# CITlabRostock/citlab-article-separation-new

Hardware: AMD Instinct MI355X
Metric: newspaper pages/sec (ARU-Net seg + GNN relation) at 3000x4500 px (higher is better)
Workload: dtype f32s

## Files before the change

### citlab-article-separation-new_amd/_lib.py

```python
import ctypes as C
import os

_HERE = os.path.dirname(os.path.abspath(__file__))
LIB_PATH = os.path.join(_HERE, "csrc", "libasep_hip.so")


class AsepError(RuntimeError):
    pass


MLP_MAX_HIDDEN = 4
ABI_VERSION = 12


class _SizedCfg(C.Structure):

    def __init__(self, *args, **kw):
        super().__init__(C.sizeof(type(self)), *args, **kw)


class AruCfg(_SizedCfg):
    _fields_ = [(n, C.c_int32) for n in (
        "struct_size", "channels", "n_classes", "feat_root", "scale_space_num", "res_depth", "num_scales_att",
        "use_attention", "mvn", "apply_softmax", "compute_dtype", "activation", "plain_u", "input_pyramid", "inp4up")]
# ... 2 lines not shown
class GnnCfg(_SizedCfg):
    _fields_ = [(n, C.c_int32) for n in (
        "struct_size", "node_feature_dim", "edge_feature_dim", "num_transition_steps", "hidden_dim", "interaction_dim",
        "interaction_hidden", "cls_hidden1", "cls_hidden2", "num_classes", "undirected_graph", "compress_input_dim", "output_type", "attention_heads", "attention_merge", "attention_hidden",
        "aggregation_type", "interaction_hidden2", "interaction_hidden3", "interaction_hidden4", "attention_hidden2", "attention_hidden3",
        "attention_hidden4", "cls_hidden3", "cls_hidden4", "lstm_use_hidden", "lstm_use_input", "visual_edge_dims")]


class ClusterSetting(C.Structure):
    _fields_ = [("min_neighbors", C.c_int32), ("assign_noise", C.c_int32), ("conf_thr", C.c_double), ("agree_thr", C.c_double)]


RESIZE_MODES = {"keep": 0, "luma": 1}
EDGE_RULES = {"bb": 0, "line": 1}
SEP_ORIENTATIONS = {None: 0, "horizontal": 1, "vertical": 2}
JPEG_ORDERS = {"gray": 0, "bgr": 1, "rgb": 2}
CLUSTER_METHODS = {"dbscan": 0, "dbscan_std": 1, "greedy": 2}


class ClusterMethodSetting(C.Structure):
    _fields_ = [("method", C.c_int32), ("count", C.c_int32), ("assign_noise", C.c_int32), ("reserved", C.c_int32),
                ("conf_thr", C.c_double), ("param", C.c_double)]


class GnnPage(C.Structure):
    _fields_ = [("N", C.c_int32), ("E", C.c_int32), ("R", C.c_int32), ("d_edges", C.c_void_p), ("d_node_feat", C.c_void_p),
                ("d_edge_feat", C.c_void_p), ("d_image", C.c_void_p), ("d_regions", C.c_void_p), ("d_num_points", C.c_void_p),
                ("d_edge_regions", C.c_void_p), ("d_edge_num_points", C.c_void_p), ("d_relations", C.c_void_p), ("d_probs_out", C.c_void_p)]


class GnnPageU8(C.Structure):
    _fields_ = [("page", GnnPage), ("d_scan", C.c_void_p), ("src_h", C.c_int32), ("src_w", C.c_int32), ("src_c", C.c_int32)]


_P = C.c_void_p
SIGNATURES = {
    "asep_device_count": (C.c_int, []),
    "asep_init": (C.c_int, [C.c_int]),
    "asep_last_error": (C.c_char_p, []),
    "asep_version": (C.c_char_p, []),
    "asep_abi_version": (C.c_int, []),
    "asep_engine_switches": (C.c_char_p, []),
    "asep_aru_load": (_P, [_P, C.c_size_t, C.POINTER(AruCfg)]),
    "asep_aru_free": (None, [_P]),
    "asep_aru_forward": (C.c_int, [_P, _P, C.c_int, C.c_int, _P, _P, _P, C.c_float]),
    "asep_aru_forward_dev": (C.c_int, [_P, _P, C.c_int, C.c_int, _P, _P, _P, C.c_float, _P]),
    "asep_aru_forward_batch_dev": (C.c_int, [_P, C.c_int, _P, C.c_int, C.c_int, _P, _P, _P, C.c_float, _P]),
    "asep_aru_trim": (C.c_int, [_P]),
    "asep_aru_forward_batch_dev2": (C.c_int, [_P, C.c_int, _P, _P, _P, _P, _P, _P, C.c_float, _P]),
    "asep_aru_get_endpoint": (C.c_long, [_P, C.c_char_p, _P, C.c_size_t, C.POINTER(C.c_int32)]),
    "asep_aru_profile": (C.c_int, [_P, C.c_int]),
    "asep_aru_profile_report": (C.c_long, [_P, C.c_char_p, C.c_size_t]),
    "asep_aru_flops": (C.c_double, [_P, C.c_int, C.c_int]),
    "asep_host_alloc": (_P, [C.c_size_t]),
    "asep_host_free": (None, [_P]),
    "asep_host_register": (C.c_int, [_P, C.c_size_t]),
    "asep_host_unregister": (C.c_int, [_P]),
    "asep_gnn_load": (_P, [_P, C.c_size_t, C.POINTER(GnnCfg)]),
    "asep_gnn_free": (None, [_P]),
    "asep_gnn_correct_edges": (C.c_int, [_P, C.c_int, C.c_int, _P, _P, _P, _P]),
    "asep_gnn_forward": (C.c_int, [_P, C.c_int, C.c_int, _P, _P, _P, C.c_int, _P, _P]),
    "asep_gnn_forward_dev": (C.c_int, [_P, C.c_int, C.c_int, _P, _P, _P, C.c_int, _P, _P, _P]),
    "asep_gnn_get_hidden": (C.c_int, [_P, _P, C.c_size_t]),
    "asep_gnn_flops": (C.c_double, [_P, C.c_int, C.c_int, C.c_int]),
    "asep_gnn_attach_backbone": (C.c_int, [_P, _P, C.c_int, C.POINTER(C.c_char_p)]),
    "asep_gnn_attach_backbone_maps": (C.c_int, [_P, _P, C.c_int, C.POINTER(C.c_char_p), C.POINTER(C.c_int32)]),
    "asep_gnn_get_feature_map": (C.c_int, [_P, C.c_int, _P, C.c_size_t, C.POINTER(C.c_int32)]),
    "asep_gnn_forward_visual": (C.c_int, [_P, C.c_int, C.c_int, _P, _P, _P, _P, C.c_int, C.c_int, _P, C.c_int, _P, _P, _P,
                                          C.c_int, _P, _P]),
    "asep_gnn_forward_visual_dev": (C.c_int, [_P, C.c_int, C.c_int, _P, _P, _P, _P, C.c_int, C.c_int, _P, C.c_int, _P, _P, _P,
                                              C.c_int, _P, _P, _P]),
    "asep_gnn_forward_visual_batch_dev": (C.c_int, [_P, C.c_int, _P, C.c_int, C.c_int, C.c_int, _P]),
    "asep_gnn_forward_visual_batch_dev2": (C.c_int, [_P, C.c_int, _P, C.POINTER(C.c_int32), C.POINTER(C.c_int32), C.c_int, _P]),
    "asep_gnn_forward_visual_batch_u8_dev": (C.c_int, [_P, C.c_int, _P, C.POINTER(C.c_int32), C.POINTER(C.c_int32), C.c_int, _P]),
    "asep_gnn_get_page_node_features": (C.c_int, [_P, C.c_int, _P, C.c_size_t]),
    "asep_gnn_get_page_feature_map": (C.c_int, [_P, C.c_int, C.c_int, _P, C.c_size_t, C.POINTER(C.c_int32)]),
    "asep_gnn_get_page_image": (C.c_int, [_P, C.c_int, _P, C.c_size_t, C.POINTER(C.c_int32)]),
    "asep_gnn_forward_batch": (C.c_int, [_P, C.c_int, C.POINTER(C.c_int32), C.POINTER(C.c_int32), C.POINTER(C.c_int32), _P, _P, _P, _P, _P,
                                         C.c_size_t]),
    "asep_gnn_forward_batch_dev": (C.c_int, [_P, C.c_int, C.POINTER(C.c_int32), C.POINTER(C.c_int32), C.POINTER(C.c_int32), _P, _P, _P, _P, _P,
                                             C.c_size_t, _P]),
    "asep_gnn_get_page_hidden": (C.c_int, [_P, C.c_int, _P, C.c_size_t]),
    "asep_gnn_get_page_edges": (C.c_int, [_P, C.c_int, _P, _P, C.c_int]),
    "asep_gnn_batch_launches": (C.c_long, [_P]),
    "asep_gnn_step_mode": (C.c_int, [_P]),
    "asep_gnn_get_node_features": (C.c_int, [_P, _P, C.c_size_t]),
    "asep_post_create": (_P, []),
    "asep_post_free": (None, [_P]),
    "asep_prep_scaled_size": (C.c_int, [C.c_int, C.c_int, C.c_double, C.POINTER(C.c_int32), C.POINTER(C.c_int32)]),
    "asep_prep_scale_gray": (C.c_int, [_P, _P, C.c_int, C.c_int, C.c_int, C.c_double, _P, _P]),
    "asep_prep_scale_gray_dev": (C.c_int, [_P, _P, C.c_int, C.c_int, C.c_int, C.c_double, _P, _P, _P]),
    "asep_prep_resize_tf1": (C.c_int, [_P, _P, C.c_int, C.c_int, C.c_int, C.c_int, C.c_int, C.c_int, _P]),
    "asep_prep_resize_tf1_dev": (C.c_int, [_P, _P, C.c_int, C.c_int, C.c_int, C.c_int, C.c_int, C.c_int, _P, _P]),
    "asep_post_cc_filter": (C.c_int, [_P, _P, C.c_int, C.c_int, C.c_int, C.c_int, C.c_int, _P]),
    "asep_post_morph_rect": (C.c_int, [_P, C.c_int, _P, C.c_int, C.c_int, C.c_int, C.c_int, _P]),
    "asep_post_separator": (C.c_int, [_P, _P, C.c_int, C.c_int, C.c_int, C.c_int, C.c_int, C.c_int, C.c_int,
                                      C.c_int, _P, _P]),
    "asep_post_separator_dev": (C.c_int, [_P, _P, C.c_int, C.c_int, C.c_int, C.c_int, C.c_int, C.c_int, C.c_int,
                                          C.c_int, _P, _P, _P]),
    "asep_post_boundary_segments": (C.c_long, [_P, _P, C.c_int, C.c_int, C.c_int, _P, _P, C.c_long]),
    "asep_post_boundary_segments_dev": (C.c_long, [_P, _P, C.c_int, C.c_int, C.c_int, _P, _P, C.c_long, _P]),
    "asep_post_boundary_segments_enqueue_dev": (C.c_int, [_P, _P, C.c_int, C.c_int, C.c_int, _P, _P, C.c_long, _P,
                                                          _P]),
    "asep_prep_gray_u8_dev": (C.c_int, [_P, _P, C.c_int, C.c_int, _P, _P]),
    "asep_post_box_sums_dev": (C.c_int, [_P, _P, C.c_int, C.c_int, C.c_int, C.c_int, C.c_int, _P, _P, _P]),
    "asep_swt_distance_transform": (C.c_int, [_P, _P, C.c_int, C.c_int, _P, C.POINTER(C.c_int32), _P]),
# ... 93 lines not shown
```

### citlab-article-separation-new_amd/csrc/aru_engine.hip

```cpp
#include <algorithm>
#include <cmath>
#include <cstdlib>
#include <memory>

#include "aru_kernels.h"
#include "res8_kernels.h"
#include "res8v_kernels.h"
#include "bf16_kernels.h"
#include "res8w_kernels.h"
#include "res8ws_kernels.h"
#include "level0_plan.h"
#include "launch_plan.h"
#include "convr_kernels.h"
#include "split_kernels.h"
#include "pyr_kernels.h"
#include "asep_common.h"
#include "aru_pack.h"

using namespace asep;

namespace {

struct Tensor {
    float* p = nullptr;
// ... 578 lines not shown
        });
    return out;
}

int grid_1d(size_t n) { return (int)std::min<size_t>((n + 255) / 256, 256 * 8); }

std::string res8_what(bool up, const TL& l) {
    return (up ? "unet_up_0 (conv1[16->8]+3xconvR+add) " : "unet_down_0 (conv1+3xconvR+add+pool) ") + dims_of(l);
}

bool r8v_fits(const TL& l) {
    for (const Tensor& t : l)
        if ((size_t)t.H * t.W >= ((size_t)1 << 28)) return false;
    return true;
}

bool r8ws_fits(const Tensor& t) { return walk_region(t.H, t.W).fits; }
bool r8ws_on(asep_aru* m) { return m->split && m->use_split_walk && m->r8_valu && m->cfg.activation == 0 && m->d_r8ws_down_w; }
const int32_t* r8ws_frame_units(asep_aru* m, const Res8Args& a, const std::vector<bool>& walk, int* count) {
    std::string key = "f";
    for (int i = 0; i < a.nprob; ++i) key += ":" + std::to_string(a.p[i].H) + "x" + std::to_string(a.p[i].W) + (walk[i] ? "w" : "t");
    std::vector<int32_t> units;
    for (int i = 0; i < a.nprob; ++i) frame_units(a.p[i].H, a.p[i].W, a.p[i].tiles_x, a.p[i].tile_begin, walk[i], R8_OW, R8_OH * R8_NP, &units);
    *count = (int)units.size();
    auto it = m->sched_cache.find(key);
    if (it != m->sched_cache.end()) return it->second;
    if (units.empty()) return nullptr;
    const int32_t* d = put_table(m, units);
    if (d) m->sched_cache[key] = d;
    return d;
}

void run_res8ws(asep_aru* m, bool up, const Res8Args& a, const std::vector<bool>& walk, const std::string& what) {
    Res8WSArgs wa{};
    int n = 0, items = 0;
    double flops = 0, bytes = 0;
    long strip_rows = 0;
    for (int i = 0; i < a.nprob; ++i) {
        if (!walk[i]) continue;
        const Res8Prob& q = a.p[i];
        Res8WSProb& p = wa.p[n++];
        if (up) { p.skip = q.img; p.dec = q.in1; }
        else { p.img = q.img; p.stats = q.stats; p.pool = q.pool; }
        p.out = q.out;
        p.H = q.H; p.W = q.W;
        const WalkRegion r = walk_region(p.H, p.W);
        p.n_strips = r.n_strips;
        p.y_end = r.y_end;
        strip_rows += (long)r.n_strips * r.rows();
        flops += 2.0 * r.pixels() * (9.0 * (up ? 16 : 1) * 8 + 3 * 9.0 * 64);
        bytes += r.pixels() * ((up ? 64.0 : 4.0) + 32.0 + (p.pool ? 8.0 : 0.0));
    }
    if (!n) return;
    const int band = walk_band(strip_rows, m->num_cus, 4);
    for (int i = 0; i < n; ++i) {
        Res8WSProb& p = wa.p[i];
        p.band = band;
        p.tile_begin = items;
        items += walk_region(p.H, p.W).items(band);
    }
    wa.nprob = n;
    if (up) { wa.b1 = m->d_r8_up_b1; wa.w1s = (const u32x4*)m->d_r8ws_up_w1; wa.ws = (const u32x4*)m->d_r8ws_up_w; wa.bias = m->d_r8_up_br; }
    else { wa.b1 = m->det_first.d_b; wa.w1f = m->det_first.d_w; wa.ws = (const u32x4*)m->d_r8ws_down_w; wa.bias = m->d_r8_down_br; }
    int units = items;
    wa.xm = oneshot_map(m, items, &units);
    ProfScope ps(m, up ? "res8ws_kernel<true>" : "res8ws_kernel<false>", flops, what);
    ps.bytes = bytes;
    if (up) hipLaunchKernelGGL(res8ws_kernel<true>, dim3(units), dim3(64), 0, m->stream, wa);
    else hipLaunchKernelGGL(res8ws_kernel<false>, dim3(units), dim3(64), 0, m->stream, wa);
}

struct Res8Kernel { void (*fn)(const Res8Args); const char* name; };
Res8Kernel res8_kernel(bool up, bool valu, int actv) {
    static const Res8Kernel k[2][4] = {
        {{res8v_down_kernel<0>, "res8v_down_kernel<0>"}, {res8v_down_kernel<1>, "res8v_down_kernel<1>"}, {res8v_down_kernel<2>, "res8v_down_kernel<2>"},
         {res8_down_kernel<false>, "res8_down_kernel<false>"}},
        {{res8v_up_kernel<0>, "res8v_up_kernel<0>"}, {res8v_up_kernel<1>, "res8v_up_kernel<1>"}, {res8v_up_kernel<2>, "res8v_up_kernel<2>"},
         {res8_up_kernel<false>, "res8_up_kernel<false>"}}};
    return k[up][valu ? actv : 3];
}

void run_res8(asep_aru* m, bool up, const TL& in0, const TL* in1, const std::vector<const float*>& stats, bool want_pool, TL* d_out, TL* pool_out) {
    for (const Tensor& t : in0) {
        d_out->push_back(new_tensor(m, t.H, t.W, 8));
        if (want_pool) pool_out->push_back(new_tensor(m, cdiv(t.H, 2), cdiv(t.W, 2), 8));
    }
    const size_t lds = up ? R8_UP_LDS : R8_DOWN_LDS;
    const char* layer = up ? "unet_up_0" : "unet_down_0";
    for_chunks<Res8Args>(in0.size(), 0.0, [&](Res8Prob& p, size_t i, Chunk& k) {
        k.bytes += tbytes(in0[i]) + (up ? tbytes((*in1)[i]) : 0.0) + tbytes((*d_out)[i]) + (want_pool ? tbytes((*pool_out)[i]) : 0.0);
        p.img = in0[i].p; p.in1 = up ? (*in1)[i].p : nullptr; p.stats = stats.empty() ? nullptr : stats[i];
        p.out = (*d_out)[i].p; p.pool = want_pool ? (*pool_out)[i].p : nullptr;
        p.H = in0[i].H; p.W = in0[i].W;
        set_tiles(p, k.units.next_tiles(p.H, p.W, R8_OW, R8_OH * R8_NP));
        k.flops += 2.0 * in0[i].H * in0[i].W * (9.0 * (up ? 16 : 1) * 8 + 3 * 9.0 * 64);
    }, [&](Res8Args& a, const Chunk& c) {
        const int tiles = c.units.total;
        const double flops = c.flops, bytes = c.bytes;
        const TL sub = c.sub(in0);
        const bool valu = m->r8_valu && r8v_fits(sub);
        if (up) { a.w1 = valu ? m->d_r8v_up_w1 : m->d_r8_up_w1; a.b1 = m->d_r8_up_b1; }
        else { a.w1 = m->det_first.d_w; a.b1 = m->det_first.d_b; }
        a.wr = (const f32x4*)(up ? (valu ? m->d_r8v_up_wr : m->d_r8_up_wr) : (valu ? m->d_r8v_down_wr : m->d_r8_down_wr));
        a.br = up ? m->d_r8_up_br : m->d_r8_down_br;
        const int actv = m->cfg.activation;
        const Res8Kernel k = res8_kernel(up, valu, actv);
        a.sched = tile_schedule(m, a, std::min(tiles, m->num_cus), R8_OH * R8_NP);
// ... 457 lines not shown
    for_chunks<TapArgs>(t.size(), 9.0 * ch * cout * 4.0, [&](TapProb& p, size_t i, Chunk& k) {
        p.img = imgs[i].p; p.t = t[i].p; p.stats = stats.empty() ? nullptr : stats[i];
        p.H = t[i].H; p.W = t[i].W;
        set_tiles(p, k.units.next_tiles(p.H, p.W, PYR_TW, PYR_TH));
        k.flops += 2.0 * t[i].H * t[i].W * 9.0 * ch * cout;
        k.bytes += tbytes(imgs[i]) + 2.0 * tbytes(t[i]);
    }, [&](TapArgs& a, const Chunk& k) {
        a.w = it->second; a.cout = cout;
        ProfScope ps(m, "pyr_tap_kernel<" + ti(ch) + ">", k.flops, layer_text(scope + " tap", k.sub(t), ch, cout));
        ps.bytes = k.bytes;
        launch_pyr_tap(m, a, ch, k.units.total);
    });
}

TL det_cnn(asep_aru* m, const TL& imgs, const std::vector<std::string>& names, const std::vector<const float*>& stats) {
    const int n = m->cfg.scale_space_num;
    std::vector<TL> skips;
    TL u = imgs;
    const bool rgb = m->det_first.cin == 3;
    const bool pyr = m->cfg.input_pyramid != 0, pyr_up = pyr && m->cfg.inp4up != 0;
    std::vector<TL> ipyr;
    if (pyr) {
        ipyr.push_back(imgs);
        for (int l = 1; l < n; ++l) ipyr.push_back(run_pool(m, ipyr.back(), rgb ? POOL_AVG_C3 : POOL_AVG_C1));
    }
    auto publish = [&](const TL& l, const std::string& suffix) {
        for (size_t i = 0; i < l.size(); ++i) m->endpoints[names[i] + suffix] = l[i];
    };
    auto first = [&](bool act) { return direct_act(m, m->det_first, imgs, act, stats); };
    auto conv = [&](const std::string& sc, const TL& in0, const TL* in1, bool act, TL* pooled = nullptr) {
        return m->bf16 ? run_convb(m, sc, in0, in1, false, act, nullptr, pooled) : conv_act(m, sc, in0, in1, false, act, nullptr, pooled);
    };
    auto deconv = [&](const std::string& sc, const TL& in, const TL& like) {
        return m->bf16 ? run_deconvb(m, sc, in, like, true) : deconv_act(m, sc, in, like);
    };
    for (int l = 0; l < n; ++l) {
        const std::string scope = "aru_net/featMapG/unet_down_" + std::to_string(l);
        const bool pool = l < n - 1;
        TL d, pooled;
        if (l == 0 && !rgb && (m->bf16 ? m->d_r8b_down_w && m->det_first.k == 3 && m->det_first.cout == 8
                                       : (m->use_fused8 || (m->fused8_var && r8v_fits(imgs))) && m->d_r8_down_wr)) {
            if (m->bf16) run_res8b(m, false, imgs, nullptr, stats, pool, &d, &pooled);
            else run_res8(m, false, imgs, nullptr, stats, pool, &d, &pooled);
        } else if (m->cfg.plain_u) {
            TL c1 = (l == 0) ? first(true) : conv(scope + "/conv1", u, nullptr, true);
            d = conv(scope + "/conv2", c1, nullptr, true, pool ? &pooled : nullptr);
        } else {
            TL t = (l == 0) ? first(false) : conv(scope + "/conv1", u, nullptr, false);
            if (pyr && l > 0) run_tap(m, scope + "/conv1", ipyr[l], t, stats);
            d = res_block_tail(m, scope, t, pool ? &pooled : nullptr);
        }
        skips.push_back(d);
        publish(d, "_unet_down_" + std::to_string(l) + "_conv");
        u = pool ? pooled : d;
    }
    for (int l = n - 2; l >= 0; --l) {
        const std::string scope = "aru_net/featMapG/unet_up_" + std::to_string(l);
        const TL& skip = skips[l];
        TL v = deconv(scope + "/deconv", u, skip);
        publish(v, "_unet_up_" + std::to_string(l) + "_deconv");
        if (l == 0 && !pyr_up && (m->bf16 ? m->d_r8b_up_w1 != nullptr : (m->use_fused8 || (m->fused8_var && r8v_fits(skip))) && m->d_r8_up_w1)) {
            TL d, none;
            if (m->bf16) run_res8b(m, true, skip, &v, {}, false, &d, &none);
            else run_res8(m, true, skip, &v, {}, false, &d, &none);
            u = d;
        } else if (m->cfg.plain_u) {
            TL c1 = conv(scope + "/conv1", skip, &v, true);
            u = conv(scope + "/conv2", c1, nullptr, true);
        } else {
            TL t = conv(scope + "/conv1", skip, &v, false);
            if (pyr_up) run_tap(m, scope + "/conv1", ipyr[l], t, stats);
            u = res_block_tail(m, scope, t);
        }
        publish(u, "_unet_up_" + std::to_string(l) + "_conv");
    }
    return u;
}

TL att_cnn(asep_aru* m, const TL& imgs, const std::vector<const float*>& stats) {
    const std::string p = "aru_net/attMapG/attPart/conv";
    TL y;
    if (m->bf16 && !m->d_att_head) { set_error("bf16 path: attention head 4x4 / 12 channels expected"); throw ArgError(); }
    const bool head_variant = m->d_att_head && !m->use_fused8 && m->fused8_wanted && m->fuse_act && m->cfg.activation != 0 && m->r8_valu && !m->bf16;
    if (m->d_att_head && (m->use_fused8 || head_variant || m->bf16)) {
        for (const Tensor& t : imgs) y.push_back(new_tensor(m, cdiv(t.H, 2), cdiv(t.W, 2), m->bf16 ? 16 : 12, m->bf16));
        bool headb = m->bf16 && m->d_att_headb && m->cfg.activation == 0;
        for (const Tensor& t : imgs) headb = headb && (size_t)t.H * t.W < ((size_t)1 << 28);
        auto fill = [&](int tw, int th) {
            return [&, tw, th](C1Prob& q, size_t i, Chunk& k) {
                k.bytes += tbytes(imgs[i]) + tbytes(y[i]);
                q.img = imgs[i].p; q.out = y[i].p; q.stats = stats.empty() ? nullptr : stats[i];
                q.H = imgs[i].H; q.W = imgs[i].W;
                set_tiles(q, k.units.next_tiles(q.H, q.W, tw, th));
                k.flops += 2.0 * imgs[i].H * imgs[i].W * 16.0 * 12;
            };
        };
        if (headb) for_chunks<AttHeadBArgs>(imgs.size(), 0.0, fill(ATTB_TW, ATTB_TH), [&](AttHeadBArgs& a, const Chunk& k) {
            a.wpk = (const u32x4*)m->d_att_headb; a.bias = m->att_first.d_b;
            int units;
            a.xm = oneshot_map(m, k.units.total, &units);
            ProfScope ps(m, "att_headb_kernel", k.flops);
            ps.bytes = k.bytes;
            hipLaunchKernelGGL(att_headb_kernel, dim3(units), dim3(256), 0, m->stream, a);
        });
        else for_chunks<AttHeadArgs>(imgs.size(), 0.0, fill(ATT_TW, ATT_TH), [&](AttHeadArgs& a, const Chunk& k) {
            a.wpk = (const f32x4*)m->d_att_head; a.bias = m->att_first.d_b; a.w = m->att_first.d_w; a.act = m->cfg.activation;
// ... 643 lines not shown
    if (!m) { set_error("asep_aru_trim: null handle"); return ASEP_ERR_ARG; }
    ASEP_HIP_CHECK(hipDeviceSynchronize());
    m->endpoints.clear();
    for (auto& Lp : m->lanes) Lp->pool.release();
    m->host_stage.release();
    m->last_nl = 0;
    return ASEP_OK;
    ASEP_GUARD_END
}

int asep_aru_profile(asep_aru* m, int enable) {
    ASEP_GUARD_BEGIN
    if (!m) { set_error("asep_aru_profile: null handle"); return ASEP_ERR_ARG; }
    m->profiling = enable != 0;
    m->prof_detail = enable == 2;
    m->prof_in_situ = enable == 3;
    if (enable) { m->prof_recs.clear(); m->ev_next = 0; m->prof_names.clear(); }
    return ASEP_OK;
    ASEP_GUARD_END
}

long asep_aru_profile_report(asep_aru* m, char* buf, size_t buflen) {
    ASEP_GUARD_BEGIN
    if (!m || !buf || buflen < 2) { set_error("asep_aru_profile_report: bad argument"); return ASEP_ERR_ARG; }
    ASEP_HIP_CHECK(hipStreamSynchronize(m->stream));
    const size_t nk = m->prof_names.size();
    std::vector<double> ms(nk, 0.0), fl(nk, 0.0), by(nk, 0.0), xf(nk, 0.0);
    std::vector<long> calls(nk, 0);
    for (const auto& r : m->prof_recs) {
        float t = 0.f;
        ASEP_HIP_CHECK(hipEventElapsedTime(&t, r.a, r.b));
        ms[r.kid] += t; fl[r.kid] += r.flops; by[r.kid] += r.bytes; xf[r.kid] += r.xflops; calls[r.kid] += 1;
    }
    std::string js = "[";
    for (size_t i = 0; i < nk; ++i) {
        if (!calls[i]) continue;
        char line[512];
        snprintf(line, sizeof(line), "%s{\"kernel\":\"%s\",\"calls\":%ld,\"total_ms\":%.6f,\"flops\":%.6e,\"bytes\":%.6e,\"executed_flops\":%.6e}",
                 js.size() > 1 ? "," : "", m->prof_names[i].c_str(), calls[i], ms[i], fl[i], by[i], xf[i]);
        js += line;
    }
    js += "]";
    if (js.size() + 1 > buflen) { set_error("asep_aru_profile_report: buffer too small (%zu needed)", js.size() + 1); return ASEP_ERR_ARG; }
    memcpy(buf, js.c_str(), js.size() + 1);
    return (long)js.size();
    ASEP_GUARD_END
}

double asep_aru_flops(const asep_aru* m, int H, int W) {
    if (!m) return 0.0;
    return flops_impl(m->cfg, H, W);
}

}

namespace {
void launch_conv_c3(asep_aru* m, const C1Args& a, int cout, bool bf, int tiles) {
    if (bf) hipLaunchKernelGGL((conv_c3_kernel<8, true>), dim3(tiles), dim3(256), 0, m->stream, a);
    else if (cout == 16) hipLaunchKernelGGL((conv_c3_kernel<16, false>), dim3(tiles), dim3(256), 0, m->stream, a);
    else hipLaunchKernelGGL((conv_c3_kernel<8, false>), dim3(tiles), dim3(256), 0, m->stream, a);
}
void launch_avgpool_c3(asep_aru* m, const PoolArgs& a, dim3 grid) { hipLaunchKernelGGL(avgpool2_cn_kernel<3>, grid, dim3(256), 0, m->stream, a); }
void launch_pyr_tap(asep_aru* m, const TapArgs& a, int ch, int tiles) {
    if (ch == 3) hipLaunchKernelGGL(pyr_tap_kernel<3>, dim3(tiles), dim3(256), pyr_tap_lds(3, a.cout), m->stream, a);
    else hipLaunchKernelGGL(pyr_tap_kernel<1>, dim3(tiles), dim3(256), pyr_tap_lds(1, a.cout), m->stream, a);
}
void launch_conv_c1_12(asep_aru* m, const C1Args& a, int tiles) { hipLaunchKernelGGL((conv_c1_kernel<3, 12>), dim3(tiles), dim3(256), 0, m->stream, a); }
void launch_combine12(const CombineArgs& ca, dim3 grid, int nsct, hipStream_t stream) {
    if (nsct == 1) hipLaunchKernelGGL((combine_kernel<12, 2, false, 1>), grid, dim3(256), 0, stream, ca);
    else hipLaunchKernelGGL((combine_kernel<12, 2, false, 0>), grid, dim3(256), 0, stream, ca);
}
}

#if defined(R8F_TRACE)
extern "C" int asep_debug_r8f_trace(int up, unsigned long long* out, int n) {
    return (int)hipMemcpyFromSymbol(out, HIP_SYMBOL(asep::g_r8f_trace), sizeof(unsigned long long) * n, (size_t)(up ? 1 : 0) * 4096 * 12 * sizeof(unsigned long long), hipMemcpyDeviceToHost);
}
#endif

#if defined(CVR_TRACE)
extern "C" int asep_debug_cvr_trace(unsigned long long* out, int n) {
    return (int)hipMemcpyFromSymbol(out, HIP_SYMBOL(asep::g_cvr_trace), sizeof(unsigned long long) * n, 0, hipMemcpyDeviceToHost);
}
#endif
#if defined(CVB_TRACE)
extern "C" int asep_debug_cvb_trace(unsigned long long* out, int n) {
    return (int)hipMemcpyFromSymbol(out, HIP_SYMBOL(asep::g_cvb_trace), sizeof(unsigned long long) * n, 0, hipMemcpyDeviceToHost);
}
#endif
```

### citlab-article-separation-new_amd/csrc/res8ws_kernels.h

```cpp
#pragma once
#include "res8w_kernels.h"
#include "split_kernels.h"

namespace asep {

struct Res8WSProb {
    const float* skip;
    const float* dec;
    const float* img;
    const float* stats;
    float* out;
    float* pool;
    int H, W;
    int n_strips;
    int band;
    int y_end;
    int tile_begin;
};
struct Res8WSArgs {
    Res8WSProb p[MAXP];
    int nprob;
    const float* b1;
    const u32x4* w1s;
    const float* w1f;
    const u32x4* ws;
    const float* bias;
    XcdMap xm;
};

__device__ __forceinline__ void r8ws_mm6(const u32x4 (&w)[3], const u32x4 (&xa)[3], const u32x4 (&xb)[3], f32x4& ca, f32x4& cb) {
    ca = mfma_bf16_k32(w[2], xa[0], ca); cb = mfma_bf16_k32(w[2], xb[0], cb);
    ca = mfma_bf16_k32(w[0], xa[2], ca); cb = mfma_bf16_k32(w[0], xb[2], cb);
    ca = mfma_bf16_k32(w[1], xa[1], ca); cb = mfma_bf16_k32(w[1], xb[1], cb);
    ca = mfma_bf16_k32(w[1], xa[0], ca); cb = mfma_bf16_k32(w[1], xb[0], cb);
    ca = mfma_bf16_k32(w[0], xa[1], ca); cb = mfma_bf16_k32(w[0], xb[1], cb);
    ca = mfma_bf16_k32(w[0], xa[0], ca); cb = mfma_bf16_k32(w[0], xb[0], cb);
}
__device__ __forceinline__ void r8ws_split4(f32x4 v, u32x2& h, u32x2& m, u32x2& l) {
    unsigned h0, m0, l0, h1, m1, l1;
    split3_pair(v.x, v.y, h0, m0, l0);
    split3_pair(v.z, v.w, h1, m1, l1);
    h = u32x2{h0, h1}; m = u32x2{m0, m1}; l = u32x2{l0, l1};
}

template <bool UP>
__global__ __launch_bounds__(64, 1) void res8ws_kernel(const Res8WSArgs a) {
    constexpr int TW = R8W_TW;
    constexpr int W0 = TW + 6, W1 = TW + 4, W2 = TW + 2;
    constexpr int NR = 4, NT = 16;
    constexpr int PL0 = W0 * 16, PL1 = W1 * 16, PL2 = W2 * 16;
    constexpr int IMB = UP ? 0 : 4 * 32 * 4;
    constexpr int R0_OFF = IMB, R1_OFF = R0_OFF + NR * 3 * PL0, R2_OFF = R1_OFF + NR * 3 * PL1, TC_OFF = R2_OFF + NR * 3 * PL2,
                  TRASH = TC_OFF + NT * TW * 32, LDSB = TRASH + 16;
    static_assert(LDSB <= 30 * 1024, "four waves per CU with room to spare");
    __shared__ __attribute__((aligned(16))) unsigned char lds[LDSB];

    const int lane = threadIdx.x;
    const int j = lane & 15, kk = lane >> 4, e = kk >> 1, ch = (kk & 1) * 4;
    const int isB = kk & 1;
    const int c = 2 * j + e;
    const int item = sched_tile(a.xm);
    if (item < 0) return;
    const int pi = prob_of_tile(a, item);
    const Res8WSProb& P = a.p[pi];
    const int li = item - P.tile_begin;
    const int bi = li / P.n_strips, si = li - bi * P.n_strips;
    const int x0 = R8W_X0 + TW * si;
    const int Ya = R8W_Y0 + bi * P.band;
    const int nb = min(P.band, P.y_end - Ya);
    const int W = P.W;

    constexpr int NF1 = UP ? 18 : 0, NFW = 27;
    u32x4 wf[NFW], w1[UP ? NF1 : 1];
    {
        const u32x4* wl = a.ws + lane;
#pragma unroll
        for (int i = 0; i < NFW; ++i) asm volatile("global_load_dwordx4 %0, %1, off" : "=a"(wf[i]) : "v"(wl + i * 64) : "memory");
        if constexpr (UP) {
            const u32x4* w1l = a.w1s + lane;
#pragma unroll
            for (int i = 0; i < NF1; ++i) asm volatile("global_load_dwordx4 %0, %1, off" : "=a"(w1[i]) : "v"(w1l + i * 64) : "memory");
        }
        asm volatile("s_waitcnt vmcnt(0)" ::: "memory");
#pragma unroll
        for (int i = 0; i < NFW; ++i) asm volatile("" : "+a"(wf[i]));
        if constexpr (UP) {
#pragma unroll
            for (int i = 0; i < NF1; ++i) asm volatile("" : "+a"(w1[i]));
        }
    }
    auto wpart = [&](int s, int ky, u32x4 (&o)[3]) {
#pragma unroll
        for (int p = 0; p < 3; ++p) o[p] = wf[(s * 3 + ky) * 3 + p];
    };
    const f32x4 bias1 = *reinterpret_cast<const f32x4*>(a.b1 + ch);
    f32x4 biasw[3];
#pragma unroll
    for (int t = 0; t < 3; ++t) biasw[t] = *reinterpret_cast<const f32x4*>(a.bias + 8 * t + ch);

    const int gxw = min(x0 - 4 + 2 * j + kk, W - 1);
    const float* __restrict__ skp = P.skip;
    const float* __restrict__ dcp = P.dec;
    auto in_row = [&](const float* __restrict__ src, int gy, f32x4& lo, f32x4& hi) {
        const float* q = src + ((size_t)gy * (size_t)W + (size_t)gxw) * 8;
        lo = *reinterpret_cast<const f32x4*>(q);
        hi = *reinterpret_cast<const f32x4*>(q + 4);
    };
    float mean = 0.f, inv = 1.f;
    if constexpr (!UP) {
        if (P.stats) { mean = P.stats[0]; inv = P.stats[1]; }
    }
    const float* __restrict__ imp = P.img;
    const size_t ioff0 = (size_t)(Ya - 4 + (lane >> 5)) * (size_t)W + (size_t)(x0 - 4 + (lane & 31));
    auto iload = [&](int p) { return imp[ioff0 + (size_t)p * 2 * (size_t)W]; };
    float* const iring = reinterpret_cast<float*>(lds);
    auto istore = [&](float v, int p) { iring[(p & 1) * 64 + lane] = (v - mean) * inv; };
    float w1v[UP ? 1 : 36];
    if constexpr (!UP) {
#pragma unroll
        for (int t = 0; t < 9; ++t)
#pragma unroll
            for (int o = 0; o < 4; ++o) w1v[t * 4 + o] = a.w1f[t * 8 + ch + o];
    }

    const int p_last = nb / 2 + 3;
    u32x4 cin[2][2][3] = {};
    f32x4 nxt[2][2][2];
    float inx = 0.f;
    if constexpr (UP) {
#pragma unroll
        for (int r = 0; r < 2; ++r) {
            f32x4 lo, hi;
            in_row(skp, Ya - 4 + r, lo, hi);
            split3_x8(lo, hi, cin[r][0][0], cin[r][0][1], cin[r][0][2]);
            in_row(dcp, Ya - 4 + r, lo, hi);
            split3_x8(lo, hi, cin[r][1][0], cin[r][1][1], cin[r][1][2]);
            in_row(skp, Ya - 2 + r, nxt[r][0][0], nxt[r][0][1]);
            in_row(dcp, Ya - 2 + r, nxt[r][1][0], nxt[r][1][1]);
        }
    } else {
        istore(iload(0), 0);
        inx = iload(1);
    }

    const int lcol = r8w_swz(2 * j + kk) * 16;
    auto whole = [&](u32x2 pa, u32x2 pb) {
        const auto s0 = __builtin_amdgcn_permlane16_swap(pa.x, pb.x, false, false);
        const auto s1 = __builtin_amdgcn_permlane16_swap(pa.y, pb.y, false, false);
        return u32x4{s0[0], s1[0], s0[1], s1[1]};
    };
    const int cs = r8w_swz(c) * 16;
    const bool v0 = j < W0 / 2, v1 = j < W1 / 2, v2 = j < W2 / 2;
    const bool tvalid = c >= 3 && c < 3 + TW;
    const int tcol = (tvalid ? c - 3 : 0) * 32 + ch * 4;
    const int trd = min(c, TW - 1) * 32 + ch * 4;
    const bool ost = j < TW / 2;
    float* __restrict__ const outp = P.out;
    float* __restrict__ const poolp = P.pool;
    const size_t Wp = (size_t)((W + 1) >> 1);

    auto store_parts = [&](f32x4 ra, f32x4 rb, int roff, int pl, bool valid, int rowa, int rowb) {
        u32x2 ha, ma, la, hb, mb, lb;
        r8ws_split4(relu4i(ra), ha, ma, la);
        r8ws_split4(relu4i(rb), hb, mb, lb);
        const u32x4 ph = whole(ha, hb), pm = whole(ma, mb), pl_ = whole(la, lb);
        const int rr = isB ? rowb : rowa;
        const int base = valid ? roff + rr * 3 * pl + cs : TRASH;
        const int step = valid ? pl : 0;
        *reinterpret_cast<u32x4*>(lds + base) = ph;
        *reinterpret_cast<u32x4*>(lds + base + step) = pm;
        *reinterpret_cast<u32x4*>(lds + base + 2 * step) = pl_;
    };
    auto ring_read = [&](int roff, int pl, int rr, u32x4 (&o)[3]) {
#pragma unroll
        for (int p = 0; p < 3; ++p) o[p] = *reinterpret_cast<const u32x4*>(lds + roff + (rr * 3 + p) * pl + lcol);
    };

    const int K = nb / 2 + 6;
#pragma unroll 1
    for (int k = 0; k < K; ++k) {
        const int i4 = (2 * k) & (NR - 1), i16 = (2 * k) & (NT - 1);
        const bool do_c1 = k < nb / 2 + 3, do_s1 = k >= 2 && k < nb / 2 + 4, do_s2 = k >= 4 && k < nb / 2 + 5, do_s3 = k >= 6;

        if (do_s3) {
            u32x4 q[4][3];
#pragma unroll
            for (int r = 0; r < 4; ++r) ring_read(R2_OFF, PL2, (i4 + r - 9) & (NR - 1), q[r]);
            const f32x4 t0 = *reinterpret_cast<const f32x4*>(lds + TC_OFF + ((i16 - 8) & (NT - 1)) * TW * 32 + trd);
            const f32x4 t1 = *reinterpret_cast<const f32x4*>(lds + TC_OFF + ((i16 - 7) & (NT - 1)) * TW * 32 + trd);
            f32x4 va = biasw[2], vb = biasw[2];
#pragma unroll
            for (int ky = 0; ky < 3; ++ky) {
                u32x4 w[3];
                wpart(2, ky, w);
                r8ws_mm6(w, q[ky], q[ky + 1], va, vb);
            }
            va = relu4i(va + t0);
            vb = relu4i(vb + t1);
            const int oy = Ya - 12 + 2 * k;
            if (ost) {
                float* o = outp + ((size_t)oy * (size_t)W + (size_t)(x0 + c)) * 8 + ch;
                *reinterpret_cast<f32x4*>(o) = va;
                *reinterpret_cast<f32x4*>(o + (size_t)W * 8) = vb;
            }
            if constexpr (!UP) {
                if (poolp) {
                    const f32x4 mv = f32x4{fmaxf(va.x, vb.x), fmaxf(va.y, vb.y), fmaxf(va.z, vb.z), fmaxf(va.w, vb.w)};
                    float pm[4];
#pragma unroll
                    for (int i = 0; i < 4; ++i) {
                        const unsigned u = __float_as_uint(mv[i]);
                        const auto s = __builtin_amdgcn_permlane32_swap(u, u, false, false);
                        pm[i] = fmaxf(__uint_as_float(s[0]), __uint_as_float(s[1]));
                    }
                    if (ost && e == 0) {
                        float* po = poolp + ((size_t)(oy >> 1) * Wp + (size_t)((x0 >> 1) + j)) * 8 + ch;
                        *reinterpret_cast<f32x4*>(po) = f32x4{pm[0], pm[1], pm[2], pm[3]};
                    }
                }
            }
        }
        if (do_s2) {
            u32x4 q[4][3];
#pragma unroll
            for (int r = 0; r < 4; ++r) ring_read(R1_OFF, PL1, (i4 + r - 6) & (NR - 1), q[r]);
            f32x4 ra = biasw[1], rb = biasw[1];
#pragma unroll
            for (int ky = 0; ky < 3; ++ky) {
                u32x4 w[3];
                wpart(1, ky, w);
                r8ws_mm6(w, q[ky], q[ky + 1], ra, rb);
            }
            store_parts(ra, rb, R2_OFF, PL2, v2, (i4 - 5) & (NR - 1), (i4 - 4) & (NR - 1));
        }
        if (do_s1) {
            u32x4 q[4][3];
#pragma unroll
            for (int r = 0; r < 4; ++r) ring_read(R0_OFF, PL0, (i4 + r - 3) & (NR - 1), q[r]);
            f32x4 ra = biasw[0], rb = biasw[0];
#pragma unroll
            for (int ky = 0; ky < 3; ++ky) {
                u32x4 w[3];
                wpart(0, ky, w);
                r8ws_mm6(w, q[ky], q[ky + 1], ra, rb);
            }
            store_parts(ra, rb, R1_OFF, PL1, v1, (i4 - 2) & (NR - 1), (i4 - 1) & (NR - 1));
        }
        if (do_c1) {
            f32x4 ra = bias1, rb = bias1;
            if constexpr (UP) {
                u32x4 x2[2][2][3];
#pragma unroll
                for (int r = 0; r < 2; ++r)
#pragma unroll
                    for (int s = 0; s < 2; ++s) split3_x8(nxt[r][s][0], nxt[r][s][1], x2[r][s][0], x2[r][s][1], x2[r][s][2]);
                if (k + 2 <= p_last) {
#pragma unroll
                    for (int r = 0; r < 2; ++r) {
                        in_row(skp, Ya + 2 * k + r, nxt[r][0][0], nxt[r][0][1]);
                        in_row(dcp, Ya + 2 * k + r, nxt[r][1][0], nxt[r][1][1]);
                    }
                }
#pragma unroll
                for (int ky = 0; ky < 3; ++ky)
#pragma unroll
                    for (int s = 0; s < 2; ++s) {
                        u32x4 w[3];
#pragma unroll
                        for (int p = 0; p < 3; ++p) w[p] = w1[(ky * 2 + s) * 3 + p];
                        u32x4 xa[3], xb[3];
#pragma unroll
                        for (int p = 0; p < 3; ++p) {
                            xa[p] = ky == 0 ? cin[0][s][p] : (ky == 1 ? cin[1][s][p] : x2[0][s][p]);
                            xb[p] = ky == 0 ? cin[1][s][p] : (ky == 1 ? x2[0][s][p] : x2[1][s][p]);
                        }
                        r8ws_mm6(w, xa, xb, ra, rb);
                    }
#pragma unroll
                for (int r = 0; r < 2; ++r)
#pragma unroll
                    for (int s = 0; s < 2; ++s)
#pragma unroll
                        for (int p = 0; p < 3; ++p) cin[r][s][p] = x2[r][s][p];
            } else {
                istore(inx, k + 1);
                if (k + 2 <= p_last) inx = iload(k + 2);
                const int cb = min(c, 29);
#pragma unroll
                for (int ky = 0; ky < 3; ++ky)
#pragma unroll
                    for (int kx = 0; kx < 3; ++kx) {
                        const float va = iring[((2 * k + ky) & 3) * 32 + cb + kx], vb = iring[((2 * k + 1 + ky) & 3) * 32 + cb + kx];
#pragma unroll
                        for (int o = 0; o < 4; ++o) {
                            ra[o] = fmaf(va, w1v[(ky * 3 + kx) * 4 + o], ra[o]);
                            rb[o] = fmaf(vb, w1v[(ky * 3 + kx) * 4 + o], rb[o]);
                        }
                    }
            }
            if (tvalid) {
                *reinterpret_cast<f32x4*>(lds + TC_OFF + ((i16 + 1) & (NT - 1)) * TW * 32 + tcol) = ra;
                *reinterpret_cast<f32x4*>(lds + TC_OFF + ((i16 + 2) & (NT - 1)) * TW * 32 + tcol) = rb;
            }
            store_parts(ra, rb, R0_OFF, PL0, v0, (i4 + 1) & (NR - 1), (i4 + 2) & (NR - 1));
        }
    }
}

}
```

### include/asep_hip.h

```cpp
#ifndef ASEP_HIP_H
#define ASEP_HIP_H

#include <stddef.h>
#include <stdint.h>

#include "asep_host_jpeg.h"

#ifdef __cplusplus
extern "C" {
#endif

#define ASEP_OK 0
#define ASEP_ERR_ARG -1
#define ASEP_ERR_HIP -2
#define ASEP_ERR_WEIGHTS -3
#define ASEP_ERR_UNSUPPORTED -4

int asep_device_count(void);
int asep_init(int device_id);
const char* asep_last_error(void);
const char* asep_version(void);
#define ASEP_ABI_VERSION 12
int asep_abi_version(void);
const char* asep_engine_switches(void);

void* asep_host_alloc(size_t nbytes);
void asep_host_free(void* p);
int asep_host_register(void* p, size_t nbytes);
int asep_host_unregister(void* p);

typedef struct asep_aru_cfg {
    int32_t struct_size;
    int32_t channels;
    int32_t n_classes;
    int32_t feat_root;
    int32_t scale_space_num;
    int32_t res_depth;
    int32_t num_scales_att;
    int32_t use_attention;
    int32_t mvn;
    int32_t apply_softmax;
    int32_t compute_dtype;
    int32_t activation;
    int32_t plain_u;
    int32_t input_pyramid;
    int32_t inp4up;
} asep_aru_cfg;

typedef struct asep_aru asep_aru;

asep_aru* asep_aru_load(const void* weight_blob, size_t nbytes, const asep_aru_cfg* cfg);
void asep_aru_free(asep_aru* m);

int asep_aru_forward(asep_aru* m, const float* img_hw, int H, int W,
                     float* out_hwc, uint8_t* out_u8, uint8_t* out_mask, float threshold);

int asep_aru_forward_dev(asep_aru* m, const float* d_img, int H, int W,
                         float* d_out, uint8_t* d_out_u8, uint8_t* d_out_mask, float threshold,
                         void* stream);

int asep_aru_forward_batch_dev(asep_aru* m, int n_pages, const float* const* d_imgs, int H, int W,
                               float* const* d_outs, uint8_t* const* d_out_u8, uint8_t* const* d_out_mask,
                               float threshold, void* stream);
int asep_aru_forward_batch_dev2(asep_aru* m, int n_pages, const float* const* d_imgs, const int32_t* H, const int32_t* W,
                                float* const* d_outs, uint8_t* const* d_out_u8, uint8_t* const* d_out_mask, float threshold,
                                void* stream);

long asep_aru_get_endpoint(asep_aru* m, const char* name, float* out, size_t max_floats, int32_t dims[3]);

int asep_aru_trim(asep_aru* m);

int asep_aru_profile(asep_aru* m, int enable);
long asep_aru_profile_report(asep_aru* m, char* buf, size_t buflen);

double asep_aru_flops(const asep_aru* m, int H, int W);

typedef struct asep_gnn_cfg {
    int32_t struct_size;
    int32_t node_feature_dim;
    int32_t edge_feature_dim;
    int32_t num_transition_steps;
    int32_t hidden_dim;
    int32_t interaction_dim;
    int32_t interaction_hidden;
    int32_t cls_hidden1;
    int32_t cls_hidden2;
    int32_t num_classes;
    int32_t undirected_graph;
    int32_t compress_input_dim;
    int32_t output_type;
    int32_t attention_heads;
    int32_t attention_merge;
    int32_t attention_hidden;
    int32_t aggregation_type;
    int32_t interaction_hidden2;
    int32_t interaction_hidden3;
    int32_t interaction_hidden4;
    int32_t attention_hidden2;
    int32_t attention_hidden3;
    int32_t attention_hidden4;
    int32_t cls_hidden3;
    int32_t cls_hidden4;
    int32_t lstm_use_hidden;
    int32_t lstm_use_input;
    int32_t visual_edge_dims;
} asep_gnn_cfg;

typedef struct asep_gnn asep_gnn;

asep_gnn* asep_gnn_load(const void* weight_blob, size_t nbytes, const asep_gnn_cfg* cfg);
void asep_gnn_free(asep_gnn* g);

int asep_gnn_correct_edges(asep_gnn* g, int N, int E, const int32_t* edges, const float* edge_feat,
                           int32_t* out_edges, float* out_feat);

int asep_gnn_forward(asep_gnn* g, int N, int E, const int32_t* edges, const float* node_feat,
                     const float* edge_feat, int R, const int32_t* relations, float* probs_out);

int asep_gnn_forward_dev(asep_gnn* g, int N, int E, const int32_t* d_edges, const float* d_node_feat,
                         const float* d_edge_feat, int R, const int32_t* d_relations, float* d_probs_out,
                         void* stream);

int asep_gnn_get_hidden(asep_gnn* g, float* out, size_t max_floats);

double asep_gnn_flops(const asep_gnn* g, int N, int E_corrected, int R);

int asep_gnn_attach_backbone(asep_gnn* g, asep_aru* backbone, int n_maps, const char* const* endpoint_names);

// ... 231 lines not shown
```

Before: 151.7.

## Recompute conv1 in down res8ws walker to shrink LDS and double occupancy

In the down variant of the res8ws walker, the conv1 output is no longer cached in an LDS tile ring. It is recomputed from a larger 16-row normalized image ring at the point of use. This frees the tile buffer, cutting the down kernel's LDS so it fits eight waves per CU instead of four, and the band sizing now uses a per-direction waves-per-CU constant. The cost is redundant 3x3 conv1 FMAs per output row. The change also adds an occupancy query entry point and publishes pooled endpoints.

```diff
diff --git a/citlab-article-separation-new_amd/_lib.py b/citlab-article-separation-new_amd/_lib.py
--- a/citlab-article-separation-new_amd/_lib.py
+++ b/citlab-article-separation-new_amd/_lib.py
@@ -78,6 +78,7 @@
     "asep_aru_profile": (C.c_int, [_P, C.c_int]),
     "asep_aru_profile_report": (C.c_long, [_P, C.c_char_p, C.c_size_t]),
     "asep_aru_flops": (C.c_double, [_P, C.c_int, C.c_int]),
+    "asep_aru_walker_occupancy": (C.c_int, [C.c_int]),
     "asep_host_alloc": (_P, [C.c_size_t]),
     "asep_host_free": (None, [_P]),
     "asep_host_register": (C.c_int, [_P, C.c_size_t]),
diff --git a/citlab-article-separation-new_amd/csrc/aru_engine.hip b/citlab-article-separation-new_amd/csrc/aru_engine.hip
--- a/citlab-article-separation-new_amd/csrc/aru_engine.hip
+++ b/citlab-article-separation-new_amd/csrc/aru_engine.hip
@@ -654,7 +654,7 @@
         bytes += r.pixels() * ((up ? 64.0 : 4.0) + 32.0 + (p.pool ? 8.0 : 0.0));
     }
     if (!n) return;
-    const int band = walk_band(strip_rows, m->num_cus, 4);
+    const int band = walk_band(strip_rows, m->num_cus, up ? R8WS_UP_WAVES_PER_CU : R8WS_DOWN_WAVES_PER_CU);
     for (int i = 0; i < n; ++i) {
         Res8WSProb& p = wa.p[i];
         p.band = band;
@@ -1218,6 +1218,7 @@
         }
         skips.push_back(d);
         publish(d, "_unet_down_" + std::to_string(l) + "_conv");
+        if (pool) publish(pooled, "_unet_down_" + std::to_string(l) + "_pool");
         u = pool ? pooled : d;
     }
     for (int l = n - 2; l >= 0; --l) {
@@ -1967,6 +1968,15 @@
     return flops_impl(m->cfg, H, W);
 }
 
+int asep_aru_walker_occupancy(int up) {
+    ASEP_GUARD_BEGIN
+    int blocks = 0;
+    if (up) { ASEP_HIP_CHECK(hipOccupancyMaxActiveBlocksPerMultiprocessor(&blocks, res8ws_kernel<true>, 64, 0)); }
+    else { ASEP_HIP_CHECK(hipOccupancyMaxActiveBlocksPerMultiprocessor(&blocks, res8ws_kernel<false>, 64, 0)); }
+    return blocks;
+    ASEP_GUARD_END
+}
+
 }
 
 namespace {
diff --git a/citlab-article-separation-new_amd/csrc/res8ws_kernels.h b/citlab-article-separation-new_amd/csrc/res8ws_kernels.h
--- a/citlab-article-separation-new_amd/csrc/res8ws_kernels.h
+++ b/citlab-article-separation-new_amd/csrc/res8ws_kernels.h
@@ -43,16 +43,19 @@
     h = u32x2{h0, h1}; m = u32x2{m0, m1}; l = u32x2{l0, l1};
 }
 
+constexpr int R8WS_UP_WAVES_PER_CU = 4, R8WS_DOWN_WAVES_PER_CU = 8;
+
 template <bool UP>
 __global__ __launch_bounds__(64, 1) void res8ws_kernel(const Res8WSArgs a) {
     constexpr int TW = R8W_TW;
     constexpr int W0 = TW + 6, W1 = TW + 4, W2 = TW + 2;
     constexpr int NR = 4, NT = 16;
+    constexpr int NI = 16;
     constexpr int PL0 = W0 * 16, PL1 = W1 * 16, PL2 = W2 * 16;
-    constexpr int IMB = UP ? 0 : 4 * 32 * 4;
-    constexpr int R0_OFF = IMB, R1_OFF = R0_OFF + NR * 3 * PL0, R2_OFF = R1_OFF + NR * 3 * PL1, TC_OFF = R2_OFF + NR * 3 * PL2,
-                  TRASH = TC_OFF + NT * TW * 32, LDSB = TRASH + 16;
-    static_assert(LDSB <= 30 * 1024, "four waves per CU with room to spare");
+    constexpr int R0_OFF = 0, R1_OFF = R0_OFF + NR * 3 * PL0, R2_OFF = R1_OFF + NR * 3 * PL1, TC_OFF = R2_OFF + NR * 3 * PL2, IM_OFF = TC_OFF,
+                  TRASH = TC_OFF + (UP ? NT * TW * 32 : NI * 32 * 4), LDSB = TRASH + 16;
+    static_assert(TRASH - TC_OFF >= (34 - W2) * 16, "the fragment reads of the last r2 plane stay inside the array");
+    static_assert(UP ? LDSB <= 30 * 1024 : LDSB <= 20 * 1024, "UP: four waves per CU with room to spare; DOWN: eight");
     __shared__ __attribute__((aligned(16))) unsigned char lds[LDSB];
 
     const int lane = threadIdx.x;
@@ -113,8 +116,8 @@
     const float* __restrict__ imp = P.img;
     const size_t ioff0 = (size_t)(Ya - 4 + (lane >> 5)) * (size_t)W + (size_t)(x0 - 4 + (lane & 31));
     auto iload = [&](int p) { return imp[ioff0 + (size_t)p * 2 * (size_t)W]; };
-    float* const iring = reinterpret_cast<float*>(lds);
-    auto istore = [&](float v, int p) { iring[(p & 1) * 64 + lane] = (v - mean) * inv; };
+    float* const iring = reinterpret_cast<float*>(lds + IM_OFF);
+    auto istore = [&](float v, int p) { iring[((2 * p) & (NI - 1)) * 32 + lane] = (v - mean) * inv; };
     float w1v[UP ? 1 : 36];
     if constexpr (!UP) {
 #pragma unroll
@@ -122,6 +125,20 @@
 #pragma unroll
             for (int o = 0; o < 4; ++o) w1v[t * 4 + o] = a.w1f[t * 8 + ch + o];
     }
+    auto conv1_down = [&](int r0, int cb, f32x4& ra, f32x4& rb) {
+        if constexpr (!UP)
+#pragma unroll
+        for (int ky = 0; ky < 3; ++ky)
+#pragma unroll
+            for (int kx = 0; kx < 3; ++kx) {
+                const float va = iring[((r0 - 1 + ky) & (NI - 1)) * 32 + cb + kx], vb = iring[((r0 + ky) & (NI - 1)) * 32 + cb + kx];
+#pragma unroll
+                for (int o = 0; o < 4; ++o) {
+                    ra[o] = fmaf(va, w1v[(ky * 3 + kx) * 4 + o], ra[o]);
+                    rb[o] = fmaf(vb, w1v[(ky * 3 + kx) * 4 + o], rb[o]);
+                }
+            }
+    };
 
     const int p_last = nb / 2 + 3;
     u32x4 cin[2][2][3] = {};
@@ -154,6 +171,7 @@
     const bool tvalid = c >= 3 && c < 3 + TW;
     const int tcol = (tvalid ? c - 3 : 0) * 32 + ch * 4;
     const int trd = min(c, TW - 1) * 32 + ch * 4;
+    const int tcb = min(c, TW - 1) + 3;
     const bool ost = j < TW / 2;
     float* __restrict__ const outp = P.out;
     float* __restrict__ const poolp = P.pool;
@@ -186,8 +204,13 @@
             u32x4 q[4][3];
 #pragma unroll
             for (int r = 0; r < 4; ++r) ring_read(R2_OFF, PL2, (i4 + r - 9) & (NR - 1), q[r]);
-            const f32x4 t0 = *reinterpret_cast<const f32x4*>(lds + TC_OFF + ((i16 - 8) & (NT - 1)) * TW * 32 + trd);
-            const f32x4 t1 = *reinterpret_cast<const f32x4*>(lds + TC_OFF + ((i16 - 7) & (NT - 1)) * TW * 32 + trd);
+            f32x4 t0 = bias1, t1 = bias1;
+            if constexpr (UP) {
+                t0 = *reinterpret_cast<const f32x4*>(lds + TC_OFF + ((i16 - 8) & (NT - 1)) * TW * 32 + trd);
+                t1 = *reinterpret_cast<const f32x4*>(lds + TC_OFF + ((i16 - 7) & (NT - 1)) * TW * 32 + trd);
+            } else {
+                conv1_down(2 * k - 8, tcb, t0, t1);
+            }
             f32x4 va = biasw[2], vb = biasw[2];
 #pragma unroll
             for (int ky = 0; ky < 3; ++ky) {
@@ -285,22 +308,13 @@
             } else {
                 istore(inx, k + 1);
                 if (k + 2 <= p_last) inx = iload(k + 2);
-                const int cb = min(c, 29);
-#pragma unroll
-                for (int ky = 0; ky < 3; ++ky)
-#pragma unroll
-                    for (int kx = 0; kx < 3; ++kx) {
-                        const float va = iring[((2 * k + ky) & 3) * 32 + cb + kx], vb = iring[((2 * k + 1 + ky) & 3) * 32 + cb + kx];
-#pragma unroll
-                        for (int o = 0; o < 4; ++o) {
-                            ra[o] = fmaf(va, w1v[(ky * 3 + kx) * 4 + o], ra[o]);
-                            rb[o] = fmaf(vb, w1v[(ky * 3 + kx) * 4 + o], rb[o]);
-                        }
-                    }
-            }
-            if (tvalid) {
-                *reinterpret_cast<f32x4*>(lds + TC_OFF + ((i16 + 1) & (NT - 1)) * TW * 32 + tcol) = ra;
-                *reinterpret_cast<f32x4*>(lds + TC_OFF + ((i16 + 2) & (NT - 1)) * TW * 32 + tcol) = rb;
+                conv1_down(2 * k + 1, min(c, 29), ra, rb);
+            }
+            if constexpr (UP) {
+                if (tvalid) {
+                    *reinterpret_cast<f32x4*>(lds + TC_OFF + ((i16 + 1) & (NT - 1)) * TW * 32 + tcol) = ra;
+                    *reinterpret_cast<f32x4*>(lds + TC_OFF + ((i16 + 2) & (NT - 1)) * TW * 32 + tcol) = rb;
+                }
             }
             store_parts(ra, rb, R0_OFF, PL0, v0, (i4 + 1) & (NR - 1), (i4 + 2) & (NR - 1));
         }
diff --git a/include/asep_hip.h b/include/asep_hip.h
--- a/include/asep_hip.h
+++ b/include/asep_hip.h
@@ -74,6 +74,8 @@
 long asep_aru_profile_report(asep_aru* m, char* buf, size_t buflen);
 
 double asep_aru_flops(const asep_aru* m, int H, int W);
+
+int asep_aru_walker_occupancy(int up);
 
 typedef struct asep_gnn_cfg {
     int32_t struct_size;
```

Measured after the change: 155.7 (median of 6 runs). 2.6% higher.
